# geopolars/geopolars

Measured on AMD Instinct MI355X. Metric: predicate evals/sec (10M pts x 1k polys point-in-polygon), higher is better.
Workload: dtype f64

## Files before the change

geopolars_amd/csrc/gpk_comm.hip:

```cpp
#include <dlfcn.h>

#include <condition_variable>
#include <mutex>
#include <vector>

#include "gpk_column.h"
#include "gpk_common.h"

extern "C" {
typedef struct gpkNcclComm* ncclComm_t;
typedef struct {
    char internal[128];
} ncclUniqueId;
typedef enum { ncclSuccess = 0 } ncclResult_t;
typedef enum { ncclInt8 = 0, ncclUint8 = 1, ncclInt32 = 2, ncclUint32 = 3, ncclInt64 = 4, ncclUint64 = 5, ncclFloat16 = 6, ncclFloat32 = 7, ncclFloat64 = 8 } ncclDataType_t;
}

namespace gpk {

struct Rccl {
    void* lib = nullptr;
    ncclResult_t (*GetUniqueId)(ncclUniqueId*) = nullptr;
    ncclResult_t (*CommInitRank)(ncclComm_t*, int, ncclUniqueId, int) = nullptr;
    ncclResult_t (*CommDestroy)(ncclComm_t) = nullptr;
// ... 88 lines not shown

namespace gpk {

struct MockWorld {
    int W = 0;
    std::mutex mu;
    std::condition_variable cv;
    int arrived = 0;
    unsigned long long gen = 0;
    const void* ptr[64];
    void meet() {
        std::unique_lock<std::mutex> lk(mu);
        const unsigned long long g = gen;
        if (++arrived == W) {
            arrived = 0;
            ++gen;
            cv.notify_all();
        } else {
            cv.wait(lk, [&] { return gen != g; });
        }
    }
};
struct MockRank {
    MockWorld* w;
    int rank;
};
static size_t mock_size(ncclDataType_t t) { return t == ncclInt64 || t == ncclUint64 || t == ncclFloat64 ? 8 : (t == ncclInt32 || t == ncclUint32 || t == ncclFloat32 ? 4 : (t == ncclFloat16 ? 2 : 1)); }
static ncclResult_t mock_all_gather(const void* send, void* recv, size_t count, ncclDataType_t t, ncclComm_t comm, hipStream_t s) {
    MockRank* m = reinterpret_cast<MockRank*>(comm);
    const size_t bytes = count * mock_size(t);
    bool ok = hipStreamSynchronize(s) == hipSuccess;
    m->w->ptr[m->rank] = send;
    m->w->meet();
    for (int k = 0; k < m->w->W; ++k) ok = ok && hipMemcpy((char*)recv + (size_t)k * bytes, m->w->ptr[k], bytes, hipMemcpyDeviceToDevice) == hipSuccess;
    m->w->meet();
    return ok ? ncclSuccess : (ncclResult_t)1;
}
static ncclResult_t mock_broadcast(const void* send, void* recv, size_t count, ncclDataType_t t, int root, ncclComm_t comm, hipStream_t s) {
    MockRank* m = reinterpret_cast<MockRank*>(comm);
    bool ok = hipStreamSynchronize(s) == hipSuccess;
    if (m->rank == root) m->w->ptr[root] = send;
    m->w->meet();
    if (recv != m->w->ptr[root]) ok = ok && hipMemcpy(recv, m->w->ptr[root], count * mock_size(t), hipMemcpyDeviceToDevice) == hipSuccess;
    m->w->meet();
    return ok ? ncclSuccess : (ncclResult_t)1;
}
static ncclResult_t mock_group() { return ncclSuccess; }
static ncclResult_t mock_destroy(ncclComm_t comm) {
    delete reinterpret_cast<MockRank*>(comm);
    return ncclSuccess;
}
static const char* mock_error(ncclResult_t) { return "in-process transport: a device copy failed"; }
static const Rccl* mock_table() {
    static const Rccl t = [] {
        Rccl r;
        r.lib = (void*)1;
        r.CommDestroy = mock_destroy;
        r.AllGather = mock_all_gather;
        r.Broadcast = mock_broadcast;
        r.GroupStart = mock_group;
        r.GroupEnd = mock_group;
        r.GetErrorString = mock_error;
        return r;
    }();
    return &t;
}

struct Shards {
    int W = 0;
    int me = -1;
    const Rccl* r = nullptr;
    gpk_comm* c = nullptr;
    const gpk_geoarray* const* local = nullptr;
    const DevGeo& mine_or(int k) const { return me < 0 ? local[k]->d : local[0]->d; }
    bool holds(int k) const { return me < 0 || k == me; }
};
// ... 379 lines not shown
```

geopolars_amd/csrc/gpk_gridindex.hip:

```cpp
#include <atomic>
#include <chrono>
#include <cmath>
#include <cstdlib>

#include "gpk_device.h"
#include "gpk_index.h"
#include "gpk_scan.h"

namespace gpk {

__global__ __launch_bounds__(256) void extent_partial_kernel(const double4* __restrict__ bbox, int64_t n, double4* __restrict__ part) {
    __shared__ double red[4][4];
    double mnx = INFINITY, mny = INFINITY, mxx = -INFINITY, mxy = -INFINITY;
    for (int64_t i = (int64_t)blockIdx.x * 256 + threadIdx.x; i < n; i += (int64_t)gridDim.x * 256) {
        const double4 b = bbox[i];
        if (b.x == b.x) {
            mnx = fmin(mnx, b.x);
            mny = fmin(mny, b.y);
            mxx = fmax(mxx, b.z);
            mxy = fmax(mxy, b.w);
        }
    }
    mnx = dev::wave_min(mnx);
    mny = dev::wave_min(mny);
// ... 94 lines not shown
        }
        items[k + 1] = key;
    }
}

static inline dim3 grid_for(int64_t n, int block) {
    int64_t b = (n + block - 1) / block;
    return dim3((unsigned)(b > 0 ? b : 1));
}

}

using namespace gpk;

extern "C" {

int32_t gpk_index_free(gpk_index* idx) {
    if (!idx) return GPK_OK;
    (void)sync_device(idx->device);
    for (int i = 0; i < 24; ++i)
        if (idx->owned[i]) cached_free(idx->owned[i]);
    delete idx;
    return GPK_OK;
}

int32_t gpk_index_describe(const gpk_index* idx, int64_t out[8]) {
    if (!idx || !out) return fail(GPK_ERR_INVALID_ARGUMENT, "NULL argument");
    for (int i = 0; i < 8; ++i) out[i] = 0;
    out[0] = idx->pip.R;
    out[1] = idx->pip_lean;
    out[2] = idx->pip.chain_xy != nullptr;
    out[3] = idx->pip.route != nullptr;
    out[4] = idx->pip_list_heavy;
    return GPK_OK;
}

int32_t gpk_index_nbytes(const gpk_index* idx, int64_t* out_bytes) {
    if (!idx || !out_bytes) return fail(GPK_ERR_INVALID_ARGUMENT, "NULL argument");
    *out_bytes = idx->nbytes;
    return GPK_OK;
}

int32_t gpk_index_build(const gpk_geoarray* a, void* stream, gpk_index** out) {
    return gpk_index_build_ex(a, GPK_INDEX_BBOX_GRID | GPK_INDEX_PIP, nullptr, stream, out);
}

int32_t gpk_index_build_ex(const gpk_geoarray* a, int32_t parts, const double* bbox4_dev, void* stream, gpk_index** out) {
    if (!a || !out) return fail(GPK_ERR_INVALID_ARGUMENT, "NULL argument");
    *out = nullptr;
    GPK_TRY(require_device());
    hipStream_t s = (hipStream_t)stream;
    const int64_t n = a->d.n_geoms;

    gpk_index* ix = new gpk_index;
    memset(ix, 0, sizeof *ix);
    ix->device = a->device;
    ix->n_geoms = n;
    ix->geom_type = a->d.type;
    ix->n_coords = a->d.n_coords;
    ix->n_rings = a->d.n_rings;
    {
        static std::atomic<uint64_t> next_serial{1};
        ix->serial = next_serial.fetch_add(1);
    }

    int gdim = (int)ceil(2.0 * sqrt((double)(n > 0 ? n : 1)));
// ... 107 lines not shown
```

geopolars_amd/csrc/gpk_index.h:

```cpp
#pragma once

#include "gpk_common.h"

namespace gpk {

struct GridParams {
    double x0, y0, inv_w, inv_h;
    int32_t gx, gy;
};

struct IndexView {
    const double4* bbox;
    const GridParams* grid;
    const int32_t* cell_off;
    const int32_t* items;
    int32_t gx, gy;
};

struct PartInfo {
    int32_t slab_base, row0 , nrows, n_rings;
};
constexpr int PIP_SUB = 8;
constexpr int PIP_SLAB_MUL = 2;
constexpr int PIP_FINE_LOG2 = 6;
__host__ __device__ inline int slab_row0_of(int32_t packed) { return packed & 0xFFFFFF; }
__host__ __device__ inline int slab_shift_of(int32_t packed) { return packed >> 24; }
constexpr uint32_t SUB_INDIRECT = 1u << 30;
struct SubCell {
    uint32_t part_flags;
    uint32_t e0, e1, e2;
    uint32_t labels[4];
};
struct SubCell2 {
    SubCell a;
    uint32_t b_part_flags;
    uint32_t b_e0, b_e1, b_e2;
    uint32_t pad[4];
};
constexpr uint32_t SUB2_BIT = 1u << 29;
constexpr int CHAIN_MAX = 12;
constexpr uint32_t HCHAIN_COUNT_MASK = 0xFu;
constexpr int HCHAIN_BASE_SHIFT = 4;
constexpr int HCHAIN_START_SHIFT = 8;
struct HalfCell {
    uint32_t lw[2];
    uint32_t part_flags;
    uint32_t aux_base;
};
static_assert(sizeof(HalfCell) * 2 == sizeof(SubCell), "two half-cell records overlay one SubCell");
static_assert(CHAIN_MAX <= (int)HCHAIN_COUNT_MASK, "the edge count of a chain is a 4-bit field");
constexpr int PIP_ROUTE_RMAX = 512;
struct RouteWord {
    uint32_t bmask;
    uint32_t gmask;
    uint32_t rec0;
    uint32_t pad;
};
struct PipView {
    int32_t R;
    double rx0, ry0, fw, fh, inv_fw, inv_fh;
    const uint32_t* cell;
    const uint32_t* list;
    const SubCell* sub;
    const SubCell2* sub2;
    const double2* chain_xy;
    const RouteWord* route;
    const SubCell* lrec;
    const uint32_t* part_geom;
    const PartInfo* part_info;
    const float4* part_box;
    const int32_t* ring_row0;
    const int32_t* ring_slab_base;
    const int32_t* slab_off;
    const double4* slab_edges;
    const int32_t* slab_vidx;
    const double2* slab_xy;
};
constexpr uint32_t CELL_TAG_EMPTY = 0u, CELL_TAG_SINGLE = 1u, CELL_TAG_LIST = 2u, CELL_TAG_SUB = 3u;

namespace dev {
__device__ __forceinline__ int cell_of(double v, double v0, double inv, int g) {
    return (int)fmin(fmax((v - v0) * inv, 0.0), (double)(g - 1));
}
}

}

struct gpk_index {
    gpk::IndexView v;
    gpk::PipView pip;
    gpk::GridParams host_grid;
    int device;
    int64_t n_geoms, n_coords, n_rings;
    int32_t geom_type;
    void* owned[24];
    int64_t nbytes;
    int32_t pip_lean;
    uint64_t serial;
    int32_t pip_list_heavy;
};

namespace gpk {
int32_t build_pip_index(const gpk_geoarray* a, gpk_index* ix, hipStream_t s, int list_records_mode = 1);
int32_t ring_bboxes(const gpk_geoarray* a, double4* out_dev, hipStream_t s);
int32_t affine_rows_impl(const gpk_geoarray* a, const double* matrices, int32_t mat_space, double* out_xy, int32_t out_space, hipStream_t s);
}
```

geopolars_amd/csrc/gpk_pipflow.hip:

```cpp
#include "gpk_pipshared.h"

namespace gpk {

constexpr int FLOW_P_MAX = 8;
constexpr int FLOW_BLOCK = 1024, FLOW_W = FLOW_BLOCK / 64;
constexpr int FLOW_ITEMS = 128;
constexpr int FLOW_PASS_AT = 40;
constexpr int FLOW_MAX_TILES = 1536;
constexpr int FLOW_ID_BITS = 22;
constexpr uint32_t FLOW_DEAD = 0xFFFFFFFFu;
constexpr uint32_t FLOW_MULTI = 0x80000000u;
constexpr uint32_t FLOW_PEND = FLOW_MULTI;
static_assert(64 * FLOW_P_MAX == 512, "an entry keeps the row within its tile in 9 bits");
static_assert(FLOW_MAX_TILES <= (1 << 14), "FlowItem::loc keeps the tile in 14 bits");

struct FlowItem {
    double px, py;
    uint32_t aux;
    uint32_t loc;
};
static_assert(sizeof(FlowItem) == 24, "list slot");

#ifdef GPK_TILE_TRACE
#define FLOW_STAMP(i)                                                                                                    \
// ... 177 lines not shown
    constexpr int S = PIP_SUB, FLOW_TILE = 64 * P, TS = P == 8 ? 9 : (P == 4 ? 8 : (P == 2 ? 7 : 6));
    static_assert(P == 1 || P == 2 || P == 4 || P == 8, "tile sizes");
    static_assert(S == 8, "the sub-cell arithmetic below is written for 8 x 8 sub-cells");
    asm volatile("" : "+v"(lane));
    const uint32_t tile = tile0 + t;
    const int64_t base = (int64_t)tile * FLOW_TILE;
    const int64_t n_points = FULL ? 0 : H_COLD(n_points);
    const uint32_t rem = FULL ? (uint32_t)FLOW_TILE : (uint32_t)(n_points - base < (int64_t)FLOW_TILE ? n_points - base : (int64_t)FLOW_TILE);
    double px[P], py[P];
    {
        const double2* __restrict__ tile_xy = h.pts_xy + base;
        static_for<P>([&](auto K) {
            constexpr int k = decltype(K)::value;
            double2 v = make_double2(NAN, NAN);
            if (FULL || ((uint32_t)(k * 64 + lane) < rem && dev::valid_row(H_COLD(pts_validity), base + k * 64 + lane))) v = dev::load_stream(tile_xy + (k * 64 + lane));
            px[k] = v.x;
            py[k] = v.y;
        });
    }
    GPK_SCHED_FENCE();
    FLOW_PHASE(1);
    const int logR = h.logR;
    const uint32_t sub_max = ((uint32_t)S << logR) - 1u;
    uint32_t sidx4[(P + 3) / 4], gw[P];
    u32x4 rec[P];
    static_for<(P + 3) / 4>([&](auto J) { sidx4[decltype(J)::value] = 0u; });
    uint32_t sxs[P], sys_[P], r0s[P];
    uint2 ms[P];
    static_for<P>([&](auto K) {
        constexpr int k = decltype(K)::value;
        uint32_t sx = cvt_u32_sat((px[k] - h.rx0) * h.inv_fw_s), sy = cvt_u32_sat((py[k] - h.ry0) * h.inv_fh_s);
        sx = sx < sub_max ? sx : sub_max;
        sy = sy < sub_max ? sy : sub_max;
        const uint32_t at = ((sy >> 3) << (logR - 5)) + (sx >> 8);
        ms[k] = s_mask[at];
        r0s[k] = s_rec0[at];
        sxs[k] = sx;
        sys_[k] = sy;
    });
    GPK_SCHED_FENCE();
    static_for<P>([&](auto K) {
        constexpr int k = decltype(K)::value;
        const uint32_t sx = sxs[k], sy = sys_[k], bit = (sx >> 3) & 31u;
        const bool real = !__builtin_isunordered(px[k], py[k]);
        const bool has = real && ((ms[k].x >> bit) & 1u) != 0u;
        const bool want = real && !has && ((ms[k].y >> bit) & 1u) != 0u;
        sidx4[k / 4] |= (((sy & 3u) << 3) | (sx & 7u)) << (8 * (k % 4));
        rec[k] = u32x4{0u, 0u, 0u, 0u};
        gw[k] = 0u;
        if (has) {
            const uint32_t w = r0s[k] + (uint32_t)__popc(__builtin_amdgcn_ubfe(ms[k].x, 0u, bit));
            rec[k] = *reinterpret_cast<const u32x4*>(h.half + (2u * w + ((sy >> 2) & 1u)));
        }
        if (want) gw[k] = h.cell[((sy >> 3) << logR) + (sx >> 3)];
    });
    GPK_SCHED_FENCE();
    FLOW_PHASE(2);
    uint32_t run = 0u, n_new = 0u;
    bool pend = false;
    uint32_t* const tile_counts = h.counts ? h.counts + base : nullptr;
    uint32_t* const tile_pool = h.pool + ((size_t)tile << TS);
    static_for<P>([&](auto K) {
        constexpr int k = decltype(K)::value;
        const uint32_t li = (uint32_t)(k * 64 + lane);
        const uint32_t s5 = (sidx4[k / 4] >> (8 * (k % 4))) & 31u;
        const uint32_t lw = (s5 & 16u) ? rec[k].y : rec[k].x;
        const uint32_t lab = (lw >> (2u * (s5 & 15u))) & 3u;
        uint32_t r = lab ? (rec[k].z & 0x3FFFFFFFu) : CODE_NONE;
        const uint32_t g = gw[k];
        const bool single = (g & 0xC0000001u) == 0x40000000u;
        if (single) r = (g >> 1) & 0x1FFFFFFFu;
        const bool walk = g != 0u && !single;
        if (!SIMPLE) {
            if (r != CODE_NONE) {
                const uint32_t geom = h.part_geom ? h.part_geom[r] : r;
                r = dev::valid_row(h.polys_validity, geom) ? geom : CODE_NONE;
            }
        }
        if (walk) r = 0u;
        const bool mine = FULL || li < rem;
        const bool cand = mine && r != CODE_NONE;
        bool listed = cand && (lab >= 2u || walk);
        const unsigned long long mcand = __ballot(cand);
        const uint32_t rank = run + lanes_below(mcand);
// ... 284 lines not shown
```

geopolars_amd/csrc/gpk_pipindex.hip:

```cpp
#include <cstdio>
#include <cstdlib>
#include <cstring>

#include <rocprim/rocprim.hpp>

#include <chrono>

#include "gpk_device.h"
#include "gpk_index.h"
#include "gpk_pip.h"
#include "gpk_scan.h"

namespace gpk {

struct FineGrid {
    int R;
    double rx0, ry0, fw, fh, inv_fw, inv_fh, pad_x, pad_y;
};
__device__ __forceinline__ int fcol(const FineGrid& f, double x) { return dev::cell_of(x, f.rx0, f.inv_fw, f.R); }
__device__ __forceinline__ int frow(const FineGrid& f, double y) { return dev::cell_of(y, f.ry0, f.inv_fh, f.R); }

__global__ void part_geom_kernel(DevGeo a, uint32_t* __restrict__ part_geom) {
    const int64_t g = (int64_t)blockIdx.x * blockDim.x + threadIdx.x;
    if (g >= a.n_geoms) return;
// ... 269 lines not shown
        if (!(cx >= bb.x && cx <= bb.z && cy >= bb.y && cy <= bb.w)) continue;
        if (!dev::valid_row(a.validity, j)) continue;
        int p0, p1;
        dev::geom_parts(a, j, p0, p1);
        for (int p = p0; p < p1; ++p) {
            flush_marks_below((unsigned long long)p);
            if (m < m_end && (marks[m] & 0xFFFFFFFFull) == (unsigned long long)p) {
                emit((uint32_t)p, 1u);
                ++m;
                continue;
            }
            if (p1 - p0 > 1) {
                int r0, r1;
                dev::part_rings(a, p, r0, r1);
                if (r1 <= r0) continue;
                const double4 rb = ring_bbox[r0];
                if (!(cx >= rb.x && cx <= rb.z && cy >= rb.y && cy <= rb.w)) continue;
            }
            const int pos = pip::part_pos_single(pv, a, p, cx, cy);
            if (pos == dev::POS_OUTSIDE) continue;
            emit((uint32_t)p, (centre_ok && pos == dev::POS_INSIDE) ? 0u : 1u);
        }
    }
    flush_marks_below(~0ull);

    if (!FILL) {
        need[c] = n >= 2 ? n + 1 : 0;
        if (n <= 1) cell[c] = n == 1 ? ((CELL_TAG_SINGLE << 30) | first_entry) : 0u;
        return;
    }
    cell[c] = (CELL_TAG_LIST << 30) | (uint32_t)list_off[c];
}

__global__ void sub_flag_kernel(const uint32_t* __restrict__ cell, const uint32_t* __restrict__ list, int64_t n_cells,
                                int32_t* __restrict__ flag, int32_t* __restrict__ flag2) {
    const int64_t c = (int64_t)blockIdx.x * blockDim.x + threadIdx.x;
    if (c >= n_cells) return;
    const uint32_t w = cell[c];
    const uint32_t tag = w >> 30;
    flag[c] = (tag == CELL_TAG_SINGLE && (w & 1u)) ? 1 : 0;
    int f2 = 0;
    if (tag == CELL_TAG_LIST) {
        const uint32_t off = w & 0x3FFFFFFFu;
        if (list[off] == 2u) f2 = (list[off + 1] & list[off + 2] & 1u) ? 1 : 0;
    }
    flag2[c] = f2;
}

__device__ __forceinline__ void record_slabs(const PipView& pv, int p, int cj, uint32_t& flags, uint32_t& e0, uint32_t& e1, uint32_t& e2) {
    const PartInfo pi = pv.part_info[p];
    e0 = e1 = e2 = 0;
    flags = (uint32_t)p | (pi.n_rings > 1 ? 0x80000000u : 0u);
    if (slab_shift_of(pi.row0) != 0) {
        flags |= SUB_INDIRECT;
        return;
    }
    const int j0 = PIP_SLAB_MUL * cj - slab_row0_of(pi.row0), j1 = j0 + 1;
    const bool lo_ok = j0 >= 0 && j0 < pi.nrows, hi_ok = j1 >= 0 && j1 < pi.nrows;
    if (lo_ok) {
        e0 = (uint32_t)pv.slab_off[pi.slab_base + j0];
        e1 = (uint32_t)pv.slab_off[pi.slab_base + j0 + 1];
        e2 = e1;
    }
    if (hi_ok) {
        if (!lo_ok) e0 = e1 = (uint32_t)pv.slab_off[pi.slab_base + j1];
        e2 = (uint32_t)pv.slab_off[pi.slab_base + j1 + 1];
    }
}
__global__ void sub_head_kernel(PipView pv, FineGrid g, const int32_t* __restrict__ work_cell, const uint32_t* __restrict__ work_part,
                                int64_t n_work, SubCell* __restrict__ sub) {
    const int64_t i = (int64_t)blockIdx.x * blockDim.x + threadIdx.x;
    if (i >= n_work) return;
    uint32_t flags, e0, e1, e2;
// ... 181 lines not shown
    drain();
    const uint32_t test_label = NP == 2 ? 3u : 2u;
    uint32_t label = test_label;
    if (!touched) {
        const double cx = g.rx0 + ((double)si + 0.5) * fw2, cy = g.ry0 + ((double)sj + 0.5) * fh2;
        const bool ok = dev::cell_of(cx, g.rx0, g.inv_fw * S, g.R * S) == si && dev::cell_of(cy, g.ry0, g.inv_fh * S, g.R * S) == sj;
        if (ok) {
            if (NP == 1) {
                const int p = pip::part_pos_single(pv, a, part[0], cx, cy);
                label = p == dev::POS_INSIDE ? 1u : (p == dev::POS_OUTSIDE ? 0u : 2u);
            } else {
                const int pa = pip::part_pos_single(pv, a, part[0], cx, cy), pb = pip::part_pos_single(pv, a, part[1], cx, cy);
                if (pa == dev::POS_BOUNDARY || pb == dev::POS_BOUNDARY)
                    label = 3u;
                else if (pa == dev::POS_INSIDE && pb == dev::POS_INSIDE)
                    label = 3u;
                else
                    label = pa == dev::POS_INSIDE ? 1u : (pb == dev::POS_INSIDE ? 2u : 0u);
            }
        }
    }
    auto slabs_of = [&](int p, uint32_t& flags, uint32_t& e0, uint32_t& e1, uint32_t& e2) { record_slabs(pv, p, cj, flags, e0, e1, e2); };
    SubCell* rec = WORK ? sub + item : (NP == 1 ? sub + pos[c] : &sub2[pos[c]].a);
    if (k == 0) {
        slabs_of(part[0], rec->part_flags, rec->e0, rec->e1, rec->e2);
        if (NP == 2) {
            SubCell2* r2 = sub2 + pos[c];
            slabs_of(part[1], r2->b_part_flags, r2->b_e0, r2->b_e1, r2->b_e2);
        }
    }
    store_labels(rec, label);
}
__global__ void sub_commit_kernel(const int32_t* __restrict__ flag, const int32_t* __restrict__ pos, const int32_t* __restrict__ flag2,
                                  const int32_t* __restrict__ pos2, int64_t n_cells, uint32_t* __restrict__ cell) {
    const int64_t c = (int64_t)blockIdx.x * blockDim.x + threadIdx.x;
    if (c >= n_cells) return;
    if (flag[c])
        cell[c] = (CELL_TAG_SUB << 30) | (uint32_t)pos[c];
    else if (flag2 && flag2[c])
        cell[c] = (CELL_TAG_SUB << 30) | SUB2_BIT | (uint32_t)pos2[c];
}

__global__ void lrec_count_kernel(const uint32_t* __restrict__ cell, const uint32_t* __restrict__ list, int64_t n_cells,
                                  int32_t* __restrict__ cnt) {
    const int64_t c = (int64_t)blockIdx.x * blockDim.x + threadIdx.x;
    if (c >= n_cells) return;
    const uint32_t w = cell[c];
    int n = 0;
    if ((w >> 30) == CELL_TAG_LIST) {
        const uint32_t off = w & 0x3FFFFFFFu, m = list[off];
        for (uint32_t t = 0; t < m; ++t) n += (int)(list[off + 1 + t] & 1u);
    }
    cnt[c] = n;
}
__device__ __forceinline__ int test_labels_of(uint32_t w) { return __popc((w >> 1) & ~w & 0x55555555u); }
__global__ void chain_xy_kernel(DevGeo a, double2* __restrict__ ext) {
    const int64_t k = (int64_t)blockIdx.x * blockDim.x + threadIdx.x;
    const int64_t n_ext = a.n_coords + a.n_rings * CHAIN_MAX;
    if (k >= n_ext) return;
    int lo = 0, hi = (int)a.n_rings - 1;
    while (lo < hi) {
        const int mid = (lo + hi + 1) >> 1;
        if ((int64_t)a.ring_off[mid] + (int64_t)mid * CHAIN_MAX <= k)
            lo = mid;
        else
            hi = mid - 1;
    }
    const int c0 = a.ring_off[lo], n = a.ring_off[lo + 1] - c0;
    const int j = (int)(k - ((int64_t)c0 + (int64_t)lo * CHAIN_MAX));
    const int ne = n - 1;
    ext[k] = n <= 0 ? make_double2(0.0, 0.0) : (ne >= 1 ? a.xy[c0 + j % ne] : a.xy[c0]);
// ... 89 lines not shown
            if (!(y >= yl && y <= yh)) break;
            lo = lo == 0 ? ne - 1 : lo - 1;
            ++len;
            ok = len <= CHAIN_MAX;
        }
        if (ok) {
            const double cx = g.rx0 + ((double)(S * ci) + 0.5 * S) * fw2;
            int wn = 0;
            bool on = false;
            if (pip::slab_range(pv, r0, row_c, e0, e1)) {
                for (int e = e0; e < e1; ++e) {
                    int dd = pip::slab_vertex(slab_vidx[e]) - c0 - lo;
                    if (dd < 0) dd += ne;
                    if (dd < len) continue;
                    const double4 ed = pip::slab_edge(pv, e);
                    on |= dev::ring_edge(ed.x, ed.y, ed.z, ed.w, cx, cy, wn);
                }
            }
            const int64_t start = (int64_t)c0 + (int64_t)r0 * CHAIN_MAX + lo;
            if (!on && wn >= -8 && wn <= 7 && start < ((int64_t)1 << (32 - HCHAIN_START_SHIFT)))
                word = (uint32_t)len | ((uint32_t)(wn & 15) << HCHAIN_BASE_SHIFT) | ((uint32_t)start << HCHAIN_START_SHIFT);
        }
    }
    hword[2 * item + half] = word;
}
__global__ void half_chain_commit_kernel(SubCell* __restrict__ sub, int64_t n_sub, const uint32_t* __restrict__ hword) {
    const int64_t i = (int64_t)blockIdx.x * blockDim.x + threadIdx.x;
    if (i >= n_sub) return;
    const SubCell rc = sub[i];
    HalfCell* h = reinterpret_cast<HalfCell*>(sub + i);
    h[0] = HalfCell{{rc.labels[0], rc.labels[1]}, rc.part_flags & ~SUB_INDIRECT, hword[2 * i]};
    h[1] = HalfCell{{rc.labels[2], rc.labels[3]}, rc.part_flags & ~SUB_INDIRECT, hword[2 * i + 1]};
}
__global__ void route_build_kernel(const uint32_t* __restrict__ cell, int64_t n_words, RouteWord* __restrict__ route) {
    const int64_t w = (int64_t)blockIdx.x * blockDim.x + threadIdx.x;
    if (w >= n_words) return;
    RouteWord rw{0u, 0u, 0u, 0u};
    bool have = false;
    for (int i = 0; i < 32; ++i) {
        const uint32_t cw = cell[32 * w + i];
        const uint32_t tag = cw >> 30, payload = cw & 0x3FFFFFFFu;
        if (tag == CELL_TAG_SUB && !(payload & SUB2_BIT)) {
            rw.bmask |= 1u << i;
            if (!have) {
                rw.rec0 = payload;
                have = true;
            }
        } else if (cw != 0u) {
            rw.gmask |= 1u << i;
        }
    }
    route[w] = rw;
}

__global__ void route_rank_kernel(RouteWord* __restrict__ route, int R) {
    const int row = blockIdx.x * blockDim.x + threadIdx.x;
    if (row >= R) return;
    const int per_row = R / 32;
    RouteWord* rw = route + (int64_t)row * per_row;
    uint32_t base = 0u;
    bool have = false;
    for (int j = 0; j < per_row; ++j) {
        if (rw[j].bmask && !have) {
            base = rw[j].rec0;
            have = true;
        }
        rw[j].pad = rw[j].bmask ? rw[j].rec0 - base : 0u;
    }
}

__global__ void sub_work_kernel(const uint32_t* __restrict__ cell, const int32_t* __restrict__ flag, const int32_t* __restrict__ pos,
                                int64_t n_cells, int32_t* __restrict__ work_cell, uint32_t* __restrict__ work_part) {
    const int64_t c = (int64_t)blockIdx.x * blockDim.x + threadIdx.x;
    if (c >= n_cells || !flag[c]) return;
    work_cell[pos[c]] = (int32_t)c;
    work_part[pos[c]] = (cell[c] & 0x3FFFFFFFu) >> 1;
}
__global__ void lrec_assign_kernel(const uint32_t* __restrict__ cell, uint32_t* __restrict__ list, int64_t n_cells,
                                   const int32_t* __restrict__ pos, int32_t* __restrict__ work_cell, uint32_t* __restrict__ work_part) {
    const int64_t c = (int64_t)blockIdx.x * blockDim.x + threadIdx.x;
    if (c >= n_cells) return;
    const uint32_t w = cell[c];
    if ((w >> 30) != CELL_TAG_LIST) return;
    const uint32_t off = w & 0x3FFFFFFFu, m = list[off];
    int32_t o = pos[c];
    for (uint32_t t = 0; t < m; ++t) {
        const uint32_t e = list[off + 1 + t];
        if (!(e & 1u)) continue;
        work_cell[o] = (int32_t)c;
        work_part[o] = e >> 1;
        list[off + 1 + t] = ((uint32_t)o << 1) | 1u;
        ++o;
    }
}

}

using namespace gpk;

namespace {
struct Temps {
    void* p[48] = {nullptr};
    int n = 0;
    double malloc_ms = 0.0;
    size_t malloc_bytes = 0;
    template <typename T>
    int32_t alloc(T** out, size_t count) {
        const size_t bytes = sizeof(T) * (count ? count : 1);
        void* q = gpk::ScratchEstimate::try_carve(gpk::workspace_aux(1), bytes);
// ... 235 lines not shown
    uint32_t* cell = nullptr;
    GPK_HIP(cached_malloc((void**)&cell, sizeof(uint32_t) * (size_t)n_cells));
    keep(cell);
    int32_t *need, *list_off;
    GPK_TRY(t.alloc(&need, (size_t)n_cells + 1));
    GPK_TRY(t.alloc(&list_off, (size_t)n_cells + 1));
    uint32_t* cell_scratch = nullptr;
    GPK_TRY(t.alloc(&cell_scratch, (size_t)n_cells * CELL_SCRATCH));
    GPK_LAUNCH("gpk_pipidx_cell_count", cell_build_kernel<false>, blocks_for(n_cells), dim3(256), 0, s, d, ix->v, pv, g, marks, mark_start,
               need, (const int32_t*)nullptr, cell, (uint32_t*)nullptr, cell_scratch, (const double4*)ring_bbox);
    GPK_TRY(exclusive_scan_i32(need, n_cells, list_off, nullptr, btot, s));
    int32_t list_len = 0;
    GPK_HIP(d2h_small(&list_len, list_off + n_cells, sizeof list_len, s));
    GPK_HIP(sync_small(s));
    if ((unsigned)list_len >= (1u << 30)) return GPK_OK;
    uint32_t* list = nullptr;
    GPK_HIP(cached_malloc((void**)&list, sizeof(uint32_t) * (size_t)(list_len ? list_len : 1)));
    keep(list);
    GPK_LAUNCH("gpk_pipidx_cell_fill", cell_build_kernel<true>, blocks_for(n_cells), dim3(256), 0, s, d, ix->v, pv, g, marks, mark_start,
               need, list_off, cell, list, cell_scratch, (const double4*)ring_bbox);
    GPK_HIP(hipStreamSynchronize(s));
    pv.cell = cell;
    pv.list = list;
    ix->pip_list_heavy = (int64_t)list_len * 4 > n_cells ? 1 : 0;

    stamp("cells");
    int32_t n_sub = 0, n_sub2 = 0;
    bool sub_overflow = false;
    int32_t* swork_cell = nullptr;
    uint32_t* swork_part = nullptr;
    SubCell* sub = nullptr;
    SubCell2* sub2 = nullptr;
    static_assert(PIP_SLAB_MUL == 2, "SubCell stores exactly two adjacent slab ranges");
    const bool level2_ok = g.pad_x / PIP_SUB > ulp64 && g.pad_y / PIP_SUB > ulp64 && R * PIP_SUB <= 32768;
    if (level2_ok) {
        int32_t *sflag, *spos, *sflag2, *spos2;
        GPK_TRY(t.alloc(&sflag, (size_t)n_cells + 1));
        GPK_TRY(t.alloc(&spos, (size_t)n_cells + 1));
        GPK_TRY(t.alloc(&sflag2, (size_t)n_cells + 1));
        GPK_TRY(t.alloc(&spos2, (size_t)n_cells + 1));
        GPK_LAUNCH("gpk_pipidx_sub_flag", sub_flag_kernel, blocks_for(n_cells), dim3(256), 0, s, cell, (const uint32_t*)list, n_cells, sflag, sflag2);
        GPK_TRY(exclusive_scan_i32(sflag, n_cells, spos, nullptr, btot, s));
        GPK_TRY(exclusive_scan_i32(sflag2, n_cells, spos2, nullptr, btot, s));
        GPK_HIP(d2h_small(&n_sub, spos + n_cells, sizeof n_sub, s));
        GPK_HIP(d2h_small(&n_sub2, spos2 + n_cells, sizeof n_sub2, s));
        GPK_HIP(sync_small(s));
        if ((unsigned)n_sub >= SUB2_BIT || (unsigned)n_sub2 >= SUB2_BIT) {
            n_sub = n_sub2 = 0;
            sub_overflow = true;
        }
        if (getenv("GPK_DEBUG_INDEX")) fprintf(stderr, "[gpk] level 2: %d one-part cells, %d two-part cells of %lld\n", n_sub, n_sub2, (long long)n_cells);
        if ((int64_t)n_sub2 < 4 * (int64_t)n_sub) n_sub2 = 0;
        if (n_sub > 0) {
            GPK_HIP(cached_malloc((void**)&sub, sizeof(SubCell) * (size_t)n_sub));
            keep(sub);
            GPK_HIP(hipMemsetAsync(sub, 0, sizeof(SubCell) * (size_t)n_sub, s));
            GPK_TRY(t.alloc(&swork_cell, (size_t)n_sub));
            GPK_TRY(t.alloc(&swork_part, (size_t)n_sub));
            GPK_LAUNCH("gpk_pipidx_sub_work", sub_work_kernel, blocks_for(n_cells), dim3(256), 0, s, (const uint32_t*)cell, (const int32_t*)sflag,
                       (const int32_t*)spos, n_cells, swork_cell, swork_part);
            GPK_LAUNCH("gpk_pipidx_sub_head", sub_head_kernel, blocks_for(n_sub), dim3(256), 0, s, pv, g, (const int32_t*)swork_cell,
                       (const uint32_t*)swork_part, (int64_t)n_sub, sub);
            if (n_refined == 0) {
                GPK_LAUNCH("gpk_pipidx_sub_build_fast", (sub_build_kernel<1, true, 1>), blocks_for((int64_t)n_sub * PIP_SUB * PIP_SUB), dim3(256), 0, s, d, pv, g,
                           (const int32_t*)nullptr, (const int32_t*)nullptr, n_cells, (const uint32_t*)cell, (const uint32_t*)list, sub, (SubCell2*)nullptr,
                           (const int32_t*)swork_cell, (const uint32_t*)swork_part, (int64_t)n_sub);
                GPK_LAUNCH("gpk_pipidx_sub_build_rest", (sub_build_kernel<1, true, 2>), blocks_for((int64_t)n_sub * PIP_SUB * PIP_SUB), dim3(256), 0, s, d, pv, g,
                           (const int32_t*)nullptr, (const int32_t*)nullptr, n_cells, (const uint32_t*)cell, (const uint32_t*)list, sub, (SubCell2*)nullptr,
                           (const int32_t*)swork_cell, (const uint32_t*)swork_part, (int64_t)n_sub);
            } else {
                GPK_LAUNCH("gpk_pipidx_sub_build", (sub_build_kernel<1, true, 0>), blocks_for((int64_t)n_sub * PIP_SUB * PIP_SUB), dim3(256), 0, s, d, pv, g,
                           (const int32_t*)nullptr, (const int32_t*)nullptr, n_cells, (const uint32_t*)cell, (const uint32_t*)list, sub, (SubCell2*)nullptr,
                           (const int32_t*)swork_cell, (const uint32_t*)swork_part, (int64_t)n_sub);
            }
        }
        if (n_sub2 > 0) {
            GPK_HIP(cached_malloc((void**)&sub2, sizeof(SubCell2) * (size_t)n_sub2));
            keep(sub2);
            GPK_HIP(hipMemsetAsync(sub2, 0, sizeof(SubCell2) * (size_t)n_sub2, s));
            GPK_LAUNCH("gpk_pipidx_sub2_build", sub_build_kernel<2>, blocks_for(n_cells * PIP_SUB * PIP_SUB), dim3(256), 0, s, d, pv, g, sflag2, spos2,
                       n_cells, (const uint32_t*)cell, (const uint32_t*)list, (SubCell*)nullptr, sub2);
        }
        if (n_sub > 0 || n_sub2 > 0) {
            GPK_LAUNCH("gpk_pipidx_sub_commit", sub_commit_kernel, blocks_for(n_cells), dim3(256), 0, s, sflag, spos, n_sub2 > 0 ? sflag2 : nullptr,
                       spos2, n_cells, cell);
            GPK_HIP(hipStreamSynchronize(s));
        }
    }
    stamp("level-2 records");
    pv.sub = sub;
    pv.sub2 = sub2;
    int32_t n_lrec = 0;
    SubCell* lrec = nullptr;
    if (level2_ok && list_len > 0 && list_records) {
        int32_t *lcnt, *lpos;
        GPK_TRY(t.alloc(&lcnt, (size_t)n_cells + 1));
        GPK_TRY(t.alloc(&lpos, (size_t)n_cells + 1));
        GPK_LAUNCH("gpk_pipidx_lrec_count", lrec_count_kernel, blocks_for(n_cells), dim3(256), 0, s, (const uint32_t*)cell, (const uint32_t*)list, n_cells,
                   lcnt);
        GPK_TRY(exclusive_scan_i32(lcnt, n_cells, lpos, nullptr, btot, s));
        GPK_HIP(d2h_small(&n_lrec, lpos + n_cells, sizeof n_lrec, s));
        GPK_HIP(sync_small(s));
        if (getenv("GPK_DEBUG_INDEX")) fprintf(stderr, "[gpk] level 2: %d boundary entries in list cells (list length %d)\n", n_lrec, list_len);
        if (n_lrec > 0 && (int64_t)n_lrec < (int64_t)1 << 28) {
            int32_t* work_cell;
            uint32_t* work_part;
            GPK_TRY(t.alloc(&work_cell, (size_t)n_lrec));
            GPK_TRY(t.alloc(&work_part, (size_t)n_lrec));
            GPK_HIP(cached_malloc((void**)&lrec, sizeof(SubCell) * (size_t)n_lrec));
            keep(lrec);
            GPK_HIP(hipMemsetAsync(lrec, 0, sizeof(SubCell) * (size_t)n_lrec, s));
            GPK_LAUNCH("gpk_pipidx_lrec_assign", lrec_assign_kernel, blocks_for(n_cells), dim3(256), 0, s, (const uint32_t*)cell, list, n_cells,
                       (const int32_t*)lpos, work_cell, work_part);
            GPK_LAUNCH("gpk_pipidx_lrec_head", sub_head_kernel, blocks_for(n_lrec), dim3(256), 0, s, pv, g, (const int32_t*)work_cell,
                       (const uint32_t*)work_part, (int64_t)n_lrec, lrec);
            if (n_refined == 0) {
                GPK_LAUNCH("gpk_pipidx_lrec_build", (sub_build_kernel<1, true, 1>), blocks_for((int64_t)n_lrec * PIP_SUB * PIP_SUB), dim3(256), 0, s, d, pv, g,
                           (const int32_t*)nullptr, (const int32_t*)nullptr, n_cells, (const uint32_t*)cell, (const uint32_t*)list, lrec, (SubCell2*)nullptr,
// ... 8 lines not shown
            }
            GPK_HIP(hipStreamSynchronize(s));
        } else {
            n_lrec = 0;
        }
    }
    stamp("list-cell records");
    pv.lrec = lrec;
    if (list_len > 0 && !lrec) {
        float4* part_box = nullptr;
        GPK_HIP(cached_malloc((void**)&part_box, sizeof(float4) * (size_t)(n_parts ? n_parts : 1)));
        keep(part_box);
        GPK_LAUNCH("gpk_pipidx_part_box", part_box_kernel, blocks_for(n_parts), dim3(256), 0, s, d, n_parts, (const double4*)ring_bbox, part_box);
        pv.part_box = part_box;
        ix->nbytes += (int64_t)(sizeof(float4) * (size_t)n_parts);
    }
    const bool boundary_cells_have_records = level2_ok && !sub_overflow && n_sub2 == 0;
    ix->pip_lean = (int64_t)list_len * 8 <= (int64_t)n_sub && n_refined == 0 && boundary_cells_have_records ? 1 : 0;
    if (getenv("GPK_DEBUG_INDEX")) fprintf(stderr, "[gpk] lean join kernel eligible: %d (list %d, refined rings: %s, one-part records %d)\n", ix->pip_lean, list_len, n_refined ? "some" : "none", n_sub);
    if (ix->pip_lean && slab_vidx && n_sub > 0 && swork_cell && d.n_coords + d.n_rings * CHAIN_MAX < ((int64_t)1 << (32 - HCHAIN_START_SHIFT))) {
        const int64_t n_ext = d.n_coords + d.n_rings * CHAIN_MAX;
        double2* cxy = nullptr;
        GPK_HIP(cached_malloc((void**)&cxy, sizeof(double2) * (size_t)n_ext));
        keep(cxy);
        uint32_t* hword;
        GPK_TRY(t.alloc(&hword, (size_t)n_sub * 2 + 2));
        pv.sub = sub;
        GPK_LAUNCH("gpk_pipidx_chain_xy", chain_xy_kernel, blocks_for(n_ext), dim3(256), 0, s, d, cxy);
        GPK_LAUNCH("gpk_pipidx_half_chain", half_chain_kernel, blocks_for((int64_t)n_sub * 2), dim3(256), 0, s, d, pv, g,
                   (const int32_t*)swork_cell, (const uint32_t*)swork_part, (int64_t)n_sub, (const int32_t*)slab_vidx, (const SubCell*)sub, hword);
        GPK_LAUNCH("gpk_pipidx_chain_commit", half_chain_commit_kernel, blocks_for(n_sub), dim3(256), 0, s, sub, (int64_t)n_sub, (const uint32_t*)hword);
        pv.chain_xy = cxy;
        ix->nbytes += (int64_t)(sizeof(double2) * (size_t)n_ext);
        if (R <= PIP_ROUTE_RMAX) {
            RouteWord* route = nullptr;
            const int64_t n_words = n_cells / 32;
            GPK_HIP(cached_malloc((void**)&route, sizeof(RouteWord) * (size_t)n_words));
            keep(route);
            GPK_LAUNCH("gpk_pipidx_route", route_build_kernel, blocks_for(n_words), dim3(256), 0, s, (const uint32_t*)cell, n_words, route);
            if (R >= 32) GPK_LAUNCH("gpk_pipidx_route_rank", route_rank_kernel, dim3((unsigned)((R + 63) / 64)), dim3(64), 0, s, route, R);
            pv.route = route;
            ix->nbytes += (int64_t)(sizeof(RouteWord) * (size_t)n_words);
        }
        GPK_HIP(hipStreamSynchronize(s));
        if (getenv("GPK_DEBUG_INDEX")) fprintf(stderr, "[gpk] half-cell chains: %d records, %lld extended coordinates%s\n", n_sub, (long long)n_ext, pv.route ? ", routing image" : "");
        stamp("local chains");
    }
    ix->nbytes += (int64_t)(sizeof(SubCell) * (size_t)n_sub + sizeof(SubCell2) * (size_t)n_sub2 + sizeof(SubCell) * (size_t)n_lrec);
    ix->pip = pv;
    ix->nbytes += (int64_t)(sizeof(uint32_t) * (size_t)n_cells + sizeof(uint32_t) * (size_t)list_len + (pv.slab_edges ? sizeof(double4) : sizeof(int32_t)) * (size_t)n_edges +
                            sizeof(int32_t) * (size_t)(n_slabs + 1) + sizeof(int32_t) * (size_t)(2 * n_rings + 1) +
                            (part_geom ? sizeof(uint32_t) * (size_t)n_parts : 0) + sizeof(PartInfo) * (size_t)n_parts);
    return GPK_OK;
}

}
```

Baseline: 112300 billion.

## Tile routing image into 8x4 cell blocks and encode interior owner per word

The routing image now covers 8x4 blocks of coarse cells instead of 32-cell row strips. Sub-cell records are renumbered in that block order, so each route word's records are contiguous and the separate rank kernel is no longer needed. Each word also stores one dominant interior polygon owner, so points in fully-inside cells resolve from the route word without loading the cell word. The mock collectives switch to async copies on the stream. This adds build complexity and owner-packing limits on record and polygon indices.

```diff
diff --git a/geopolars_amd/csrc/gpk_comm.hip b/geopolars_amd/csrc/gpk_comm.hip
--- a/geopolars_amd/csrc/gpk_comm.hip
+++ b/geopolars_amd/csrc/gpk_comm.hip
@@ -144,7 +144,8 @@
     bool ok = hipStreamSynchronize(s) == hipSuccess;
     m->w->ptr[m->rank] = send;
     m->w->meet();
-    for (int k = 0; k < m->w->W; ++k) ok = ok && hipMemcpy((char*)recv + (size_t)k * bytes, m->w->ptr[k], bytes, hipMemcpyDeviceToDevice) == hipSuccess;
+    for (int k = 0; k < m->w->W; ++k) ok = ok && hipMemcpyAsync((char*)recv + (size_t)k * bytes, m->w->ptr[k], bytes, hipMemcpyDeviceToDevice, s) == hipSuccess;
+    ok = hipStreamSynchronize(s) == hipSuccess && ok;
     m->w->meet();
     return ok ? ncclSuccess : (ncclResult_t)1;
 }
@@ -153,7 +154,8 @@
     bool ok = hipStreamSynchronize(s) == hipSuccess;
     if (m->rank == root) m->w->ptr[root] = send;
     m->w->meet();
-    if (recv != m->w->ptr[root]) ok = ok && hipMemcpy(recv, m->w->ptr[root], count * mock_size(t), hipMemcpyDeviceToDevice) == hipSuccess;
+    if (recv != m->w->ptr[root]) ok = ok && hipMemcpyAsync(recv, m->w->ptr[root], count * mock_size(t), hipMemcpyDeviceToDevice, s) == hipSuccess;
+    ok = hipStreamSynchronize(s) == hipSuccess && ok;
     m->w->meet();
     return ok ? ncclSuccess : (ncclResult_t)1;
 }
diff --git a/geopolars_amd/csrc/gpk_gridindex.hip b/geopolars_amd/csrc/gpk_gridindex.hip
--- a/geopolars_amd/csrc/gpk_gridindex.hip
+++ b/geopolars_amd/csrc/gpk_gridindex.hip
@@ -150,6 +150,8 @@
     out[2] = idx->pip.chain_xy != nullptr;
     out[3] = idx->pip.route != nullptr;
     out[4] = idx->pip_list_heavy;
+    out[5] = idx->route_own;
+    out[6] = idx->route_single;
     return GPK_OK;
 }
 
diff --git a/geopolars_amd/csrc/gpk_index.h b/geopolars_amd/csrc/gpk_index.h
--- a/geopolars_amd/csrc/gpk_index.h
+++ b/geopolars_amd/csrc/gpk_index.h
@@ -1,6 +1,7 @@
 #pragma once
 
 #include "gpk_common.h"
+#include "gpk_route.h"
 
 namespace gpk {
 
@@ -49,13 +50,6 @@
 };
 static_assert(sizeof(HalfCell) * 2 == sizeof(SubCell), "two half-cell records overlay one SubCell");
 static_assert(CHAIN_MAX <= (int)HCHAIN_COUNT_MASK, "the edge count of a chain is a 4-bit field");
-constexpr int PIP_ROUTE_RMAX = 512;
-struct RouteWord {
-    uint32_t bmask;
-    uint32_t gmask;
-    uint32_t rec0;
-    uint32_t pad;
-};
 struct PipView {
     int32_t R;
     double rx0, ry0, fw, fh, inv_fw, inv_fh;
@@ -98,6 +92,7 @@
     int32_t pip_lean;
     uint64_t serial;
     int32_t pip_list_heavy;
+    int32_t route_own, route_single;
 };
 
 namespace gpk {
diff --git a/geopolars_amd/csrc/gpk_pipflow.hip b/geopolars_amd/csrc/gpk_pipflow.hip
--- a/geopolars_amd/csrc/gpk_pipflow.hip
+++ b/geopolars_amd/csrc/gpk_pipflow.hip
@@ -233,7 +233,7 @@
         uint32_t sx = cvt_u32_sat((px[k] - h.rx0) * h.inv_fw_s), sy = cvt_u32_sat((py[k] - h.ry0) * h.inv_fh_s);
         sx = sx < sub_max ? sx : sub_max;
         sy = sy < sub_max ? sy : sub_max;
-        const uint32_t at = ((sy >> 3) << (logR - 5)) + (sx >> 8);
+        const uint32_t at = route_block_sub(sx, sy, logR);
         ms[k] = s_mask[at];
         r0s[k] = s_rec0[at];
         sxs[k] = sx;
@@ -242,15 +242,17 @@
     GPK_SCHED_FENCE();
     static_for<P>([&](auto K) {
         constexpr int k = decltype(K)::value;
-        const uint32_t sx = sxs[k], sy = sys_[k], bit = (sx >> 3) & 31u;
+        const uint32_t sx = sxs[k], sy = sys_[k], bit = route_bit_sub(sx, sy);
         const bool real = !__builtin_isunordered(px[k], py[k]);
-        const bool has = real && ((ms[k].x >> bit) & 1u) != 0u;
-        const bool want = real && !has && ((ms[k].y >> bit) & 1u) != 0u;
+        const uint32_t recs = ms[k].x & ~ms[k].y;
+        const bool b = ((ms[k].x >> bit) & 1u) != 0u, g = ((ms[k].y >> bit) & 1u) != 0u;
+        const bool has = real && b && !g;
+        const bool want = real && g && !b;
         sidx4[k / 4] |= (((sy & 3u) << 3) | (sx & 7u)) << (8 * (k % 4));
         rec[k] = u32x4{0u, 0u, 0u, 0u};
-        gw[k] = 0u;
+        gw[k] = real && b && g ? (CELL_TAG_SINGLE << 30) | (route_owner(r0s[k]) << 1) : 0u;
         if (has) {
-            const uint32_t w = r0s[k] + (uint32_t)__popc(__builtin_amdgcn_ubfe(ms[k].x, 0u, bit));
+            const uint32_t w = route_rec0(r0s[k]) + (uint32_t)__popc(__builtin_amdgcn_ubfe(recs, 0u, bit));
             rec[k] = *reinterpret_cast<const u32x4*>(h.half + (2u * w + ((sy >> 2) & 1u)));
         }
         if (want) gw[k] = h.cell[((sy >> 3) << logR) + (sx >> 3)];
diff --git a/geopolars_amd/csrc/gpk_pipindex.hip b/geopolars_amd/csrc/gpk_pipindex.hip
--- a/geopolars_amd/csrc/gpk_pipindex.hip
+++ b/geopolars_amd/csrc/gpk_pipindex.hip
@@ -325,13 +325,14 @@
     cell[c] = (CELL_TAG_LIST << 30) | (uint32_t)list_off[c];
 }
 
-__global__ void sub_flag_kernel(const uint32_t* __restrict__ cell, const uint32_t* __restrict__ list, int64_t n_cells,
+__device__ __forceinline__ int64_t sub_slot(int64_t c, int route_logR) { return route_logR ? (int64_t)route_order((uint32_t)c, route_logR) : c; }
+__global__ void sub_flag_kernel(const uint32_t* __restrict__ cell, const uint32_t* __restrict__ list, int64_t n_cells, int route_logR,
                                 int32_t* __restrict__ flag, int32_t* __restrict__ flag2) {
     const int64_t c = (int64_t)blockIdx.x * blockDim.x + threadIdx.x;
     if (c >= n_cells) return;
     const uint32_t w = cell[c];
     const uint32_t tag = w >> 30;
-    flag[c] = (tag == CELL_TAG_SINGLE && (w & 1u)) ? 1 : 0;
+    flag[sub_slot(c, route_logR)] = (tag == CELL_TAG_SINGLE && (w & 1u)) ? 1 : 0;
     int f2 = 0;
     if (tag == CELL_TAG_LIST) {
         const uint32_t off = w & 0x3FFFFFFFu;
@@ -579,11 +580,12 @@
     store_labels(rec, label);
 }
 __global__ void sub_commit_kernel(const int32_t* __restrict__ flag, const int32_t* __restrict__ pos, const int32_t* __restrict__ flag2,
-                                  const int32_t* __restrict__ pos2, int64_t n_cells, uint32_t* __restrict__ cell) {
+                                  const int32_t* __restrict__ pos2, int64_t n_cells, int route_logR, uint32_t* __restrict__ cell) {
     const int64_t c = (int64_t)blockIdx.x * blockDim.x + threadIdx.x;
     if (c >= n_cells) return;
-    if (flag[c])
-        cell[c] = (CELL_TAG_SUB << 30) | (uint32_t)pos[c];
+    const int64_t o = sub_slot(c, route_logR);
+    if (flag[o])
+        cell[c] = (CELL_TAG_SUB << 30) | (uint32_t)pos[o];
     else if (flag2 && flag2[c])
         cell[c] = (CELL_TAG_SUB << 30) | SUB2_BIT | (uint32_t)pos2[c];
 }
@@ -739,49 +741,60 @@
     h[0] = HalfCell{{rc.labels[0], rc.labels[1]}, rc.part_flags & ~SUB_INDIRECT, hword[2 * i]};
     h[1] = HalfCell{{rc.labels[2], rc.labels[3]}, rc.part_flags & ~SUB_INDIRECT, hword[2 * i + 1]};
 }
-__global__ void route_build_kernel(const uint32_t* __restrict__ cell, int64_t n_words, RouteWord* __restrict__ route) {
+__global__ void route_build_kernel(const uint32_t* __restrict__ cell, int64_t n_words, int logR, RouteWord* __restrict__ route,
+                                   uint32_t* __restrict__ counters) {
     const int64_t w = (int64_t)blockIdx.x * blockDim.x + threadIdx.x;
     if (w >= n_words) return;
-    RouteWord rw{0u, 0u, 0u, 0u};
-    bool have = false;
-    for (int i = 0; i < 32; ++i) {
-        const uint32_t cw = cell[32 * w + i];
-        const uint32_t tag = cw >> 30, payload = cw & 0x3FFFFFFFu;
+    const uint32_t bx = (uint32_t)w & ((1u << (logR - 3)) - 1u), by = (uint32_t)w >> (logR - 3);
+    uint32_t cw[32];
+#pragma unroll
+    for (int i = 0; i < 32; ++i) cw[i] = cell[((int64_t)((by << 2) | (uint32_t)(i >> 3)) << logR) + ((bx << 3) | (uint32_t)(i & 7))];
+    uint32_t rec = 0u, other = 0u, inside = 0u, rec0 = 0u;
+#pragma unroll
+    for (int i = 31; i >= 0; --i) {
+        const uint32_t tag = cw[i] >> 30, payload = cw[i] & 0x3FFFFFFFu;
         if (tag == CELL_TAG_SUB && !(payload & SUB2_BIT)) {
-            rw.bmask |= 1u << i;
-            if (!have) {
-                rw.rec0 = payload;
-                have = true;
-            }
-        } else if (cw != 0u) {
-            rw.gmask |= 1u << i;
-        }
-    }
-    route[w] = rw;
-}
-
-__global__ void route_rank_kernel(RouteWord* __restrict__ route, int R) {
-    const int row = blockIdx.x * blockDim.x + threadIdx.x;
-    if (row >= R) return;
-    const int per_row = R / 32;
-    RouteWord* rw = route + (int64_t)row * per_row;
-    uint32_t base = 0u;
-    bool have = false;
-    for (int j = 0; j < per_row; ++j) {
-        if (rw[j].bmask && !have) {
-            base = rw[j].rec0;
-            have = true;
-        }
-        rw[j].pad = rw[j].bmask ? rw[j].rec0 - base : 0u;
+            rec |= 1u << i;
+            rec0 = payload;
+        } else if ((cw[i] & 0xC0000001u) == (CELL_TAG_SINGLE << 30)) {
+            inside |= 1u << i;
+        } else if (cw[i] != 0u) {
+            other |= 1u << i;
+        }
+    }
+    uint32_t owner = ROUTE_NO_OWNER, own = 0u;
+    if (inside) {
+        uint32_t left = inside;
+#pragma unroll
+        for (int i = 0; i < 32; ++i) {
+            if (!((left >> i) & 1u)) continue;
+            const uint32_t p = (cw[i] >> 1) & 0x1FFFFFFFu;
+            uint32_t m = 0u;
+#pragma unroll
+            for (int j = i; j < 32; ++j) m |= (uint32_t)(((cw[j] >> 1) & 0x1FFFFFFFu) == p) << j;
+            m &= left;
+            left &= ~m;
+            if (p < ROUTE_OWNER_MAX && (__popc(m) > __popc(own) || (__popc(m) == __popc(own) && p < owner))) {
+                owner = p;
+                own = m;
+            }
+        }
+    }
+    route[w] = RouteWord{rec | own, other | inside, route_pack(rec0, owner), 0u};
+    if (inside) {
+        if (own) atomicAdd(&counters[0], (uint32_t)__popc(own));
+        atomicAdd(&counters[1], (uint32_t)__popc(inside));
     }
 }
 
 __global__ void sub_work_kernel(const uint32_t* __restrict__ cell, const int32_t* __restrict__ flag, const int32_t* __restrict__ pos,
-                                int64_t n_cells, int32_t* __restrict__ work_cell, uint32_t* __restrict__ work_part) {
+                                int64_t n_cells, int route_logR, int32_t* __restrict__ work_cell, uint32_t* __restrict__ work_part) {
     const int64_t c = (int64_t)blockIdx.x * blockDim.x + threadIdx.x;
-    if (c >= n_cells || !flag[c]) return;
-    work_cell[pos[c]] = (int32_t)c;
-    work_part[pos[c]] = (cell[c] & 0x3FFFFFFFu) >> 1;
+    if (c >= n_cells) return;
+    const int64_t o = sub_slot(c, route_logR);
+    if (!flag[o]) return;
+    work_cell[pos[o]] = (int32_t)c;
+    work_part[pos[o]] = (cell[c] & 0x3FFFFFFFu) >> 1;
 }
 __global__ void lrec_assign_kernel(const uint32_t* __restrict__ cell, uint32_t* __restrict__ list, int64_t n_cells,
                                    const int32_t* __restrict__ pos, int32_t* __restrict__ work_cell, uint32_t* __restrict__ work_part) {
@@ -1083,6 +1096,9 @@
     SubCell* sub = nullptr;
     SubCell2* sub2 = nullptr;
     static_assert(PIP_SLAB_MUL == 2, "SubCell stores exactly two adjacent slab ranges");
+    int route_logR = 0;
+    if (R <= PIP_ROUTE_RMAX)
+        while ((1 << route_logR) < R) ++route_logR;
     const bool level2_ok = g.pad_x / PIP_SUB > ulp64 && g.pad_y / PIP_SUB > ulp64 && R * PIP_SUB <= 32768;
     if (level2_ok) {
         int32_t *sflag, *spos, *sflag2, *spos2;
@@ -1090,7 +1106,8 @@
         GPK_TRY(t.alloc(&spos, (size_t)n_cells + 1));
         GPK_TRY(t.alloc(&sflag2, (size_t)n_cells + 1));
         GPK_TRY(t.alloc(&spos2, (size_t)n_cells + 1));
-        GPK_LAUNCH("gpk_pipidx_sub_flag", sub_flag_kernel, blocks_for(n_cells), dim3(256), 0, s, cell, (const uint32_t*)list, n_cells, sflag, sflag2);
+        GPK_LAUNCH("gpk_pipidx_sub_flag", sub_flag_kernel, blocks_for(n_cells), dim3(256), 0, s, cell, (const uint32_t*)list, n_cells, route_logR, sflag,
+                   sflag2);
         GPK_TRY(exclusive_scan_i32(sflag, n_cells, spos, nullptr, btot, s));
         GPK_TRY(exclusive_scan_i32(sflag2, n_cells, spos2, nullptr, btot, s));
         GPK_HIP(d2h_small(&n_sub, spos + n_cells, sizeof n_sub, s));
@@ -1109,7 +1126,7 @@
             GPK_TRY(t.alloc(&swork_cell, (size_t)n_sub));
             GPK_TRY(t.alloc(&swork_part, (size_t)n_sub));
             GPK_LAUNCH("gpk_pipidx_sub_work", sub_work_kernel, blocks_for(n_cells), dim3(256), 0, s, (const uint32_t*)cell, (const int32_t*)sflag,
-                       (const int32_t*)spos, n_cells, swork_cell, swork_part);
+                       (const int32_t*)spos, n_cells, route_logR, swork_cell, swork_part);
             GPK_LAUNCH("gpk_pipidx_sub_head", sub_head_kernel, blocks_for(n_sub), dim3(256), 0, s, pv, g, (const int32_t*)swork_cell,
                        (const uint32_t*)swork_part, (int64_t)n_sub, sub);
             if (n_refined == 0) {
@@ -1134,7 +1151,7 @@
         }
         if (n_sub > 0 || n_sub2 > 0) {
             GPK_LAUNCH("gpk_pipidx_sub_commit", sub_commit_kernel, blocks_for(n_cells), dim3(256), 0, s, sflag, spos, n_sub2 > 0 ? sflag2 : nullptr,
-                       spos2, n_cells, cell);
+                       spos2, n_cells, route_logR, cell);
             GPK_HIP(hipStreamSynchronize(s));
         }
     }
@@ -1209,17 +1226,24 @@
         GPK_LAUNCH("gpk_pipidx_chain_commit", half_chain_commit_kernel, blocks_for(n_sub), dim3(256), 0, s, sub, (int64_t)n_sub, (const uint32_t*)hword);
         pv.chain_xy = cxy;
         ix->nbytes += (int64_t)(sizeof(double2) * (size_t)n_ext);
+        uint32_t route_host[2] = {0u, 0u};
         if (R <= PIP_ROUTE_RMAX) {
             RouteWord* route = nullptr;
             const int64_t n_words = n_cells / 32;
             GPK_HIP(cached_malloc((void**)&route, sizeof(RouteWord) * (size_t)n_words));
             keep(route);
-            GPK_LAUNCH("gpk_pipidx_route", route_build_kernel, blocks_for(n_words), dim3(256), 0, s, (const uint32_t*)cell, n_words, route);
-            if (R >= 32) GPK_LAUNCH("gpk_pipidx_route_rank", route_rank_kernel, dim3((unsigned)((R + 63) / 64)), dim3(64), 0, s, route, R);
+            uint32_t* route_counts;
+            GPK_TRY(t.alloc(&route_counts, 2));
+            GPK_HIP(hipMemsetAsync(route_counts, 0, 2 * sizeof(uint32_t), s));
+            GPK_LAUNCH("gpk_pipidx_route", route_build_kernel, blocks_for(n_words), dim3(256), 0, s, (const uint32_t*)cell, n_words, route_logR, route,
+                       route_counts);
+            GPK_HIP(d2h_small(route_host, route_counts, sizeof route_host, s));
             pv.route = route;
             ix->nbytes += (int64_t)(sizeof(RouteWord) * (size_t)n_words);
         }
-        GPK_HIP(hipStreamSynchronize(s));
+        GPK_HIP(sync_small(s));
+        ix->route_own = (int32_t)route_host[0];
+        ix->route_single = (int32_t)route_host[1];
         if (getenv("GPK_DEBUG_INDEX")) fprintf(stderr, "[gpk] half-cell chains: %d records, %lld extended coordinates%s\n", n_sub, (long long)n_ext, pv.route ? ", routing image" : "");
         stamp("local chains");
     }
diff --git a/geopolars_amd/csrc/gpk_route.h b/geopolars_amd/csrc/gpk_route.h
--- /dev/null
+++ b/geopolars_amd/csrc/gpk_route.h
@@ -0,0 +1,42 @@
+#pragma once
+
+#include <cstdint>
+
+#if defined(__HIPCC__)
+#define GPK_ROUTE_FN __host__ __device__ inline
+#else
+#define GPK_ROUTE_FN inline
+#endif
+
+namespace gpk {
+
+constexpr int PIP_ROUTE_RMAX = 512;
+struct RouteWord {
+    uint32_t bmask;
+    uint32_t gmask;
+    uint32_t rec0;
+    uint32_t pad;
+};
+
+constexpr int ROUTE_REC_BITS = 18;
+constexpr uint32_t ROUTE_REC_MASK = (1u << ROUTE_REC_BITS) - 1u;
+constexpr uint32_t ROUTE_OWNER_MAX = (1u << (32 - ROUTE_REC_BITS)) - 1u;
+constexpr uint32_t ROUTE_NO_OWNER = 0xFFFFFFFFu;
+static_assert(PIP_ROUTE_RMAX * PIP_ROUTE_RMAX == 1 << ROUTE_REC_BITS, "a record index of an imaged raster fits the field");
+
+GPK_ROUTE_FN uint32_t route_pack(uint32_t rec0, uint32_t owner) {
+    return (rec0 & ROUTE_REC_MASK) | (owner < ROUTE_OWNER_MAX ? (owner + 1u) << ROUTE_REC_BITS : 0u);
+}
+GPK_ROUTE_FN uint32_t route_rec0(uint32_t packed) { return packed & ROUTE_REC_MASK; }
+GPK_ROUTE_FN uint32_t route_owner(uint32_t packed) { return (packed >> ROUTE_REC_BITS) - 1u; }
+
+GPK_ROUTE_FN uint32_t route_block(uint32_t cx, uint32_t cy, int logR) { return ((cy >> 2) << (logR - 3)) + (cx >> 3); }
+GPK_ROUTE_FN uint32_t route_bit(uint32_t cx, uint32_t cy) { return ((cy & 3u) << 3) | (cx & 7u); }
+GPK_ROUTE_FN uint32_t route_block_sub(uint32_t sx, uint32_t sy, int logR) { return ((sy >> 5) << (logR - 3)) + (sx >> 6); }
+GPK_ROUTE_FN uint32_t route_bit_sub(uint32_t sx, uint32_t sy) { return ((sy >> 3) & 3u) << 3 | ((sx >> 3) & 7u); }
+GPK_ROUTE_FN uint32_t route_order(uint32_t c, int logR) {
+    const uint32_t cx = c & ((1u << logR) - 1u), cy = c >> logR;
+    return (route_block(cx, cy, logR) << 5) | route_bit(cx, cy);
+}
+
+}
```

New measurement: 126600 billion (median of 6 runs). 1.13x the previous value.
